# Viictor/vrenderer

Hardware: AMD Instinct MI355X
Metric: shaded Gpixels/s at 8K terrain (higher is better)
Workload: dtype f32

## Files before the change

include/vrterrain.h:

```cpp
#ifndef VRTERRAIN_H
#define VRTERRAIN_H

#include <stddef.h>
#include <stdint.h>

#ifdef __cplusplus
extern "C" {
#endif

#define VR_API __attribute__((visibility("default")))

enum {
    VR_OK = 0,
    VR_ERR_INVALID_ARGUMENT = 1,
    VR_ERR_NO_DEVICE = 2,
    VR_ERR_OUT_OF_MEMORY = 3,
    VR_ERR_TOO_MANY_INSTANCES = 4,
    VR_ERR_OVERFLOW = 5,
    VR_ERR_HIP = 6
};

#define VR_MAX_LODS 12

typedef struct vr_terrain_params {
// ... 236 lines not shown
    const vr_light*         lights;
    int32_t                 num_lights;
    int32_t                 tiled;
    float                   ambient_top[3], ambient_bottom[3];
    const vr_shadow_binding* shadow;
    vr_image*               hdr_out;
    struct vr_tonemap*      tonemap;
    const vr_tonemap_params* tonemap_params;
    float                   frame_time_seconds;
    int32_t                 reserved0;
    void*                   ldr_out;
    size_t                  ldr_capacity;
    void*                   nccl_comm;
    void*                   gathered;
    void*                   ldr_frame;
} vr_frame_desc;
VR_API int vr_frame_submit(vr_terrain* t, vr_gbuffer* gb, const vr_frame_desc* frame);

VR_API int vr_synth_heightmap(vr_context* ctx, int32_t size, uint32_t seed, uint8_t* out_r8);
VR_API int vr_synth_albedo(vr_context* ctx, int32_t size, uint32_t seed,
                           const uint8_t* height_r8, uint8_t* out_srgba8);

VR_API int vr_debug_render_stats(vr_terrain* t, uint32_t out[8]);
VR_API int vr_debug_tile_order(vr_terrain* t, int32_t* out_tiles, uint32_t* out_bin_lengths, int32_t capacity, int32_t* out_count);
VR_API int vr_terrain_memory_bytes(const vr_terrain* t, uint64_t out[4]);
VR_API int vr_debug_download_vertices(vr_terrain* t, uint32_t first, uint32_t count, float* out_xyzw_wxwz);
VR_API int vr_debug_srgb_encode(vr_context* ctx, const float* in, size_t n, uint8_t* out);
VR_API int vr_debug_fastmath_check(vr_context* ctx, unsigned long long out[3]);

#ifdef __cplusplus
}
#endif
#endif
```

vrenderer_amd/capi.py:

```python
import ctypes as C
import os

VR_MAX_LODS = 12
VR_OWNER_TILE = 128

VR_OK = 0
VR_ERR_INVALID_ARGUMENT = 1
VR_ERR_NO_DEVICE = 2
VR_ERR_OUT_OF_MEMORY = 3
VR_ERR_TOO_MANY_INSTANCES = 4
VR_ERR_OVERFLOW = 5
VR_ERR_HIP = 6

VR_LIGHT_DIRECTIONAL = 1
VR_LIGHT_SPOT = 2
VR_LIGHT_POINT = 3
VR_K_COUNT = 19
VR_TONEMAP_BINS = 256
VR_OPT_ASYNC_GEOMETRY = 1
VR_OPT_DISPATCH_EVENTS = 2
VR_OPT_RASTER_TILE = 3
VR_OPT_PLANE_TRACKING = 4
VR_OPT_SCRATCH_WORST_CASE = 5

# ... 101 lines not shown


assert C.sizeof(Instance) == 112
assert C.sizeof(Light) == 64
assert C.sizeof(FrameDesc) == 160

_PKG_DIR = os.path.dirname(os.path.abspath(__file__))
LIB_PATH = os.path.join(_PKG_DIR, "lib", "libvrterrain.so")
if os.environ.get("VRTERRAIN_LIB"):
    LIB_PATH = os.environ["VRTERRAIN_LIB"]

EXPORTS = [
    "vr_context_create", "vr_context_destroy", "vr_context_set_stream", "vr_context_set_option", "vr_context_synchronize",
    "vr_last_error", "vr_version", "vr_build_experiments", "vr_timing_enable", "vr_timing_collect", "vr_timing_kernel_count", "vr_kernel_name", "vr_view_from_camera", "vr_terrain_default_params",
    "vr_render_default_params", "vr_terrain_create", "vr_terrain_destroy", "vr_terrain_num_lods",
    "vr_terrain_lod_ranges", "vr_terrain_download_mip", "vr_terrain_update_heights", "vr_terrain_download_node_heights", "vr_terrain_select", "vr_terrain_render", "vr_terrain_render_lit", "vr_terrain_prepare", "vr_terrain_num_chunks",
    "vr_gbuffer_create", "vr_gbuffer_destroy", "vr_gbuffer_clear", "vr_gbuffer_describe", "vr_gbuffer_plane_known_zero", "vr_gbuffer_region_census",
    "vr_gbuffer_download", "vr_gbuffer_upload", "vr_image_create", "vr_image_destroy",
    "vr_image_device_ptr", "vr_image_download", "vr_image_upload", "vr_ldr_image_create", "vr_ldr_image_destroy", "vr_ldr_image_device_ptr", "vr_ldr_image_capacity", "vr_ldr_image_download", "vr_ldr_image_upload", "vr_deferred_light", "vr_deferred_light_tiled", "vr_deferred_tiled_status", "vr_partition_num_tiles",
    "vr_partition_packed_bytes", "vr_partition_prepare", "vr_frame_detile",
    "vr_shadow_default_params", "vr_shadow_view_setup", "vr_deferred_light_shadowed",
    "vr_tonemap_default_params", "vr_tonemap_create", "vr_tonemap_destroy", "vr_tonemap_reset_exposure", "vr_tonemap_reset_histogram",
    "vr_tonemap_add_frame_to_histogram", "vr_tonemap_histogram_device_ptr", "vr_tonemap_compute_exposure", "vr_tonemap_render",
    "vr_tonemap_simple_render", "vr_tonemap_download", "vr_partition_packed_bytes_ldr", "vr_frame_detile_ldr", "vr_frame_submit", "vr_frame_allgather", "vr_frame_allgather_tiles", "vr_frame_allgather_ldr", "vr_tonemap_allreduce_histogram", "vr_synth_heightmap", "vr_synth_albedo", "vr_debug_srgb_encode", "vr_debug_fastmath_check", "vr_debug_render_stats", "vr_debug_tile_order", "vr_debug_download_vertices", "vr_terrain_memory_bytes",
]

_lib = None


def load_library():
    global _lib
    if _lib is not None:
        return _lib
    if not os.path.exists(LIB_PATH):
        raise RuntimeError(
            f"{LIB_PATH} is missing: the HIP extension has not been built "
            "(run `python -c 'import __graft_entry__ as g; g.build()'`). "
            "vrenderer_amd has no CPU fallback.")
    try:
        import torch
    except Exception:
        pass
    lib = C.CDLL(LIB_PATH, mode=C.RTLD_GLOBAL)
    P = C.POINTER
    vp = C.c_void_p
    sig = {
        "vr_context_create": (C.c_int, [C.c_int, P(vp)]),
# ... 63 lines not shown
        "vr_shadow_default_params": (None, [P(ShadowParams), C.c_float]),
        "vr_shadow_view_setup": (C.c_int, [P(Light), P(View), P(ShadowParams), P(View)]),
        "vr_deferred_light_shadowed": (C.c_int, [vp, P(View), vp, P(Light), C.c_int32, P(C.c_float), P(C.c_float),
                                                 vp, P(Partition), P(ShadowBinding)]),
        "vr_tonemap_default_params": (None, [P(TonemapParams)]),
        "vr_tonemap_create": (C.c_int, [vp, P(vp)]),
        "vr_tonemap_destroy": (None, [vp]),
        "vr_tonemap_reset_exposure": (C.c_int, [vp, C.c_float]),
        "vr_tonemap_reset_histogram": (C.c_int, [vp]),
        "vr_tonemap_add_frame_to_histogram": (C.c_int, [vp, P(TonemapParams), vp, C.c_int32, C.c_int32, P(Partition)]),
        "vr_tonemap_histogram_device_ptr": (vp, [vp]),
        "vr_tonemap_compute_exposure": (C.c_int, [vp, P(TonemapParams), C.c_float]),
        "vr_tonemap_render": (C.c_int, [vp, P(TonemapParams), vp, C.c_int32, C.c_int32, vp, C.c_size_t, P(Partition)]),
        "vr_tonemap_simple_render": (C.c_int, [vp, P(TonemapParams), C.c_float, vp, vp, C.c_size_t]),
        "vr_tonemap_download": (C.c_int, [vp, P(C.c_uint32), P(C.c_float)]),
        "vr_partition_packed_bytes_ldr": (C.c_size_t, [C.c_int32, C.c_int32, C.c_int32]),
        "vr_frame_detile_ldr": (C.c_int, [vp, vp, C.c_int32, C.c_int32, C.c_int32, vp]),
        "vr_synth_heightmap": (C.c_int, [vp, C.c_int32, C.c_uint32, vp]),
        "vr_synth_albedo": (C.c_int, [vp, C.c_int32, C.c_uint32, vp, vp]),
        "vr_debug_srgb_encode": (C.c_int, [vp, vp, C.c_size_t, vp]),
        "vr_debug_fastmath_check": (C.c_int, [vp, vp]),
        "vr_debug_render_stats": (C.c_int, [vp, P(C.c_uint32)]),
        "vr_debug_tile_order": (C.c_int, [vp, vp, vp, C.c_int32, P(C.c_int32)]),
        "vr_debug_download_vertices": (C.c_int, [vp, C.c_uint32, C.c_uint32, vp]),
        "vr_terrain_memory_bytes": (C.c_int, [vp, P(C.c_uint64)]),
    }
    for name in EXPORTS:
        fn = getattr(lib, name)
        fn.restype, fn.argtypes = sig[name]
    _lib = lib
    return lib


class VrError(RuntimeError):
    def __init__(self, code, where):
        msg = ""
        try:
            msg = load_library().vr_last_error().decode()
        except Exception:
            pass
        super().__init__(f"{where} failed with status {code}: {msg}")
        self.code = code


def check(code, where):
    if code != VR_OK:
# ... 2 lines not shown
```

vrenderer_amd/csrc/vr_deferred.hip:

```cpp
#include "vr_internal.h"
#include "vr_tex_dev.h"

#include <math.h>
#include <string.h>

#include "vr_deferred_dev.h"

template <bool PACKED, bool NT = false>
__device__ __forceinline__ void store_quad(uint2* __restrict__ out, size_t out_index, const uint32_t o[8])
{
    if (PACKED) {
        uint2* dst = reinterpret_cast<uint2*>(reinterpret_cast<uint16_t*>(out) + out_index * 3);
        dst[0] = make_uint2(o[0], (o[1] & 0xffffu) | (o[2] << 16));
        dst[1] = make_uint2((o[2] >> 16) | (o[3] << 16), o[4]);
        dst[2] = make_uint2((o[5] & 0xffffu) | (o[6] << 16), (o[6] >> 16) | (o[7] << 16));
    } else {
        uint4* dst = reinterpret_cast<uint4*>(out + out_index);
        if (NT) {
            typedef uint32_t u32x4 __attribute__((ext_vector_type(4)));
            const u32x4 v0 = { o[0], o[1], o[2], o[3] }, v1 = { o[4], o[5], o[6], o[7] };
            __builtin_nontemporal_store(v0, reinterpret_cast<u32x4*>(dst)); __builtin_nontemporal_store(v1, reinterpret_cast<u32x4*>(dst) + 1);
        } else {
            dst[0] = make_uint4(o[0], o[1], o[2], o[3]);
            dst[1] = make_uint4(o[4], o[5], o[6], o[7]);
// ... 41 lines not shown
    const uint4 df = LD16(g_diff + p);
    const uint4 sp = LD16(g_spec + p);
    const uint4 n0 = LD16(g_nrm + p);
    const uint4 n1 = LD16(g_nrm + p + 2);
    const uint4 e0 = LD16(g_emi + p);
    const uint4 e1 = LD16(g_emi + p + 2);
#undef LD16

    const float depth[4] = { dz.x, dz.y, dz.z, dz.w };
    const uint32_t dfa[4] = { df.x, df.y, df.z, df.w }, spa[4] = { sp.x, sp.y, sp.z, sp.w };
    const uint32_t na[8] = { n0.x, n0.y, n0.z, n0.w, n1.x, n1.y, n1.z, n1.w };
    const uint32_t ea[8] = { e0.x, e0.y, e0.z, e0.w, e1.x, e1.y, e1.z, e1.w };
    uint32_t o[8];
#pragma unroll
    for (int k = 0; k < 4; k++) {
        float rgb[3];
        shade_pixel<EXTRA, SHADOW>(a, lut, px0 + k, py, depth[k], dfa[k], spa[k], na[2 * k], na[2 * k + 1], ea[2 * k], ea[2 * k + 1], rgb, &sh);
        o[2 * k] = vr_float_to_half(rgb[0]) | (vr_float_to_half(rgb[1]) << 16);
        o[2 * k + 1] = vr_float_to_half(rgb[2]);
    }
    store_quad<PACKED, NT>(out, out_index, o);
}

template <bool PACKED, bool EXTRA, bool SHADOW = false, bool NT = false>
__global__ __launch_bounds__(256, VR_DEFERRED_WAVES) void k_deferred(DeferredArgs a, const float* __restrict__ g_depth,
                                                   const uint32_t* __restrict__ g_diff, const uint32_t* __restrict__ g_spec,
                                                   const uint2* __restrict__ g_nrm, const uint2* __restrict__ g_emi,
                                                   uint2* __restrict__ out, const float* __restrict__ lut_g,
                                                   const int32_t* __restrict__ owned_tiles, ShadowArgs sh, PlaneHints hints)
{
    __shared__ float lut[256];
    int px0, py;
    size_t out_index;
    bool valid;
    if (PACKED) {
        const int lt = blockIdx.x >> 4, rg = blockIdx.x & 15;
        const int tile = owned_tiles[lt];
        const int ty = tile / a.tiles_x, tx = tile - ty * a.tiles_x;
        const int row = rg * 8 + (threadIdx.x >> 5), col = (threadIdx.x & 31) * 4;
        px0 = tx * VR_OWNER_TILE + col; py = ty * VR_OWNER_TILE + row;
        out_index = ((size_t)lt * VR_OWNER_TILE + row) * VR_OWNER_TILE + col;
        valid = px0 < a.w && py < a.h;
    } else {
        const size_t q = (size_t)blockIdx.x * 256 + threadIdx.x;
        const size_t p = q * 4;
        valid = p < (size_t)a.w * a.h;
        py = (int)(p / (size_t)a.w); px0 = (int)(p - (size_t)py * a.w);
        out_index = p;
    }
    const size_t p = (size_t)py * a.w + px0;
    uint32_t st = 0u;
    if (valid && hints.region != nullptr) st = hints.region[((size_t)(py >> 5) * hints.tiles32_x + (size_t)(px0 >> 5)) * 4 + (size_t)((py & 31) >> 3)];
    const float lut_r = lut_g[threadIdx.x];
    typedef uint32_t u32x4 __attribute__((ext_vector_type(4)));
#define LD16(ptr) ({ u32x4 v_; if (NT) v_ = __builtin_nontemporal_load(reinterpret_cast<const u32x4*>(ptr)); else v_ = *reinterpret_cast<const u32x4*>(ptr); \
                     make_uint4(v_.x, v_.y, v_.z, v_.w); })
    const bool known_clear = st == kRegionClear, known_spec = st == kRegionSpec;
    uint4 dzu = make_uint4(0x3f800000u, 0x3f800000u, 0x3f800000u, 0x3f800000u), df = make_uint4(0u, 0u, 0u, 0u), n0 = df, n1 = df, e0 = df, e1 = df;
    uint4 sp = known_spec ? make_uint4(hints.spec_const, hints.spec_const, hints.spec_const, hints.spec_const) : df;
    if (valid && !known_clear) {
        dzu = LD16(g_depth + p);
        df = LD16(g_diff + p);
        if (!known_spec) sp = LD16(g_spec + p);
        n0 = LD16(g_nrm + p);
        n1 = LD16(g_nrm + p + 2);
        if (!hints.emissive_zero) { e0 = LD16(g_emi + p); e1 = LD16(g_emi + p + 2); }
    }
    lut[threadIdx.x] = lut_r;
    __syncthreads();
    if (!valid) return;
    {
        const uint32_t any = (dzu.x ^ 0x3f800000u) | (dzu.y ^ 0x3f800000u) | (dzu.z ^ 0x3f800000u) | (dzu.w ^ 0x3f800000u)
                           | df.x | df.y | df.z | df.w | sp.x | sp.y | sp.z | sp.w | n0.x | n0.y | n0.z | n0.w | n1.x | n1.y | n1.z | n1.w
                           | e0.x | e0.y | e0.z | e0.w | e1.x | e1.y | e1.z | e1.w;
        if (__all(any == 0u)) {
            const uint32_t z[8] = { 0u, 0u, 0u, 0u, 0u, 0u, 0u, 0u };
            store_quad<PACKED, NT>(out, out_index, z);
            return;
        }
    }
    const float4 dz = make_float4(__uint_as_float(dzu.x), __uint_as_float(dzu.y), __uint_as_float(dzu.z), __uint_as_float(dzu.w));
#undef LD16

    const float depth[4] = { dz.x, dz.y, dz.z, dz.w };
    const uint32_t dfa[4] = { df.x, df.y, df.z, df.w }, spa[4] = { sp.x, sp.y, sp.z, sp.w };
    const uint32_t na[8] = { n0.x, n0.y, n0.z, n0.w, n1.x, n1.y, n1.z, n1.w };
    const uint32_t ea[8] = { e0.x, e0.y, e0.z, e0.w, e1.x, e1.y, e1.z, e1.w };
    uint32_t o[8];
#pragma unroll
    for (int k = 0; k < 4; k++) {
        float rgb[3];
        shade_pixel<EXTRA, SHADOW>(a, lut, px0 + k, py, depth[k], dfa[k], spa[k], na[2 * k], na[2 * k + 1], ea[2 * k], ea[2 * k + 1], rgb, &sh);
        o[2 * k] = vr_float_to_half(rgb[0]) | (vr_float_to_half(rgb[1]) << 16);
        o[2 * k + 1] = vr_float_to_half(rgb[2]);
// ... 66 lines not shown
        VR_REQUIRE(shadow->light_index >= 0 && shadow->light_index < num_lights, "shadow light_index out of range");
        VR_REQUIRE(lights[shadow->light_index].type == VR_LIGHT_DIRECTIONAL, "only a directional light carries the cascaded shadow map");
        VR_REQUIRE(shadow->shadow_map->w == shadow->shadow_map->h && shadow->shadow_map->w == shadow->light_view->viewport_w
                   && shadow->light_view->viewport_h == shadow->light_view->viewport_w, "shadow map must be square and match the light view's viewport");
        VR_REQUIRE(shadow->shadow_map->ctx->device == ctx->device, "shadow map lives on another device");
        for (int i = 0; i < 16; i++) sh.w2c[i] = shadow->light_view->world_to_clip[i];
        { VR_HIP(hipSetDevice(ctx->device)); const int rc = vr_gbuffer_materialise(shadow->shadow_map, ctx->stream); if (rc) return rc; }
        sh.depth = shadow->shadow_map->depth; sh.res = shadow->shadow_map->w; sh.light_index = shadow->light_index;
        sh.bias = shadow->depth_bias; sh.out_of_bounds = lights[shadow->light_index].out_of_bounds_shadow;
    }
    VR_REQUIRE(num_lights >= 0 && num_lights <= kMaxLights, "at most 16 lights (terrain_cb.h:15)");
    VR_REQUIRE(num_lights == 0 || lights, "lights is NULL");
    VR_REQUIRE(view->viewport_w == gb->w && view->viewport_h == gb->h && view->viewport_x == 0 && view->viewport_y == 0,
               "view viewport must cover the G-buffer");
    VR_HIP(hipSetDevice(ctx->device));
    DeferredArgs a;
    bool extra = false;
    { int rc = vr_deferred_make_args(view, gb->w, gb->h, lights, num_lights, amb_top, amb_bottom, &a, &extra); if (rc) return rc; }
    const size_t npx = (size_t)gb->w * gb->h;
    const bool packed = part != nullptr;
    PlaneHints hints;
    { int rc = vr_gbuffer_plane_hints(gb, ctx->stream, &hints); if (rc) return rc; }
    const bool hinted = hints.region != nullptr || hints.emissive_zero != 0;
    VrKernelScope ks(ctx, VR_K_DEFERRED, ctx->stream, true);
    if (packed) {
        const PartTables* pt = nullptr;
        int rc = vr_partition_tables(ctx, gb->w, gb->h, part, &pt);
        if (rc) return rc;
        VR_REQUIRE((size_t)pt->max_owned * VR_OWNER_TILE * VR_OWNER_TILE * 6 <= hdr->capacity_bytes,
                   "hdr_out is smaller than vr_partition_packed_bytes()");
        VR_REQUIRE(gb->w % 4 == 0, "partitioned frames need a width that is a multiple of 4");
        a.tiles_x = (gb->w + VR_OWNER_TILE - 1) / VR_OWNER_TILE;
        if (pt->num_owned > 0) {
            if (!hinted) {
                auto kern = shadow ? k_deferred_stream<true, true, true> : (extra ? k_deferred_stream<true, true> : k_deferred_stream<true, false>);
                VR_LAUNCH_TIMED(ks, kern, dim3((unsigned)pt->num_owned * 16), dim3(256), ctx->stream, a, gb->depth, gb->diffuse,
                                   gb->specular, gb->normals, gb->emissive, (uint2*)hdr->data, ctx->d_srgb_lut, pt->d_owned_tiles, sh);
            } else {
            auto kern = shadow ? k_deferred<true, true, true> : (extra ? k_deferred<true, true> : k_deferred<true, false>);
            VR_LAUNCH_TIMED(ks, kern, dim3((unsigned)pt->num_owned * 16), dim3(256), ctx->stream, a, gb->depth, gb->diffuse,
                               gb->specular, gb->normals, gb->emissive, (uint2*)hdr->data, ctx->d_srgb_lut, pt->d_owned_tiles, sh, hints);
            }
        }
    } else {
        VR_REQUIRE(npx * 8 <= hdr->capacity_bytes, "hdr_out is smaller than the frame");
        if (gb->w % 4 == 0) {
            const size_t quads = npx / 4;
            const bool nt = true;
            if (!hinted) {
                auto kern = shadow ? k_deferred_stream<false, true, true, true> : extra ? k_deferred_stream<false, true, false, true>
                                                                                        : k_deferred_stream<false, false, false, true>;
                VR_LAUNCH_TIMED(ks, kern, dim3((unsigned)((quads + 255) / 256)), dim3(256), ctx->stream, a, gb->depth, gb->diffuse,
                                   gb->specular, gb->normals, gb->emissive, (uint2*)hdr->data, ctx->d_srgb_lut, (const int32_t*)nullptr, sh);
            } else {
            auto kern = shadow ? (nt ? k_deferred<false, true, true, true> : k_deferred<false, true, true, false>)
                               : extra ? (nt ? k_deferred<false, true, false, true> : k_deferred<false, true, false, false>)
                                       : (nt ? k_deferred<false, false, false, true> : k_deferred<false, false, false, false>);
            VR_LAUNCH_TIMED(ks, kern, dim3((unsigned)((quads + 255) / 256)), dim3(256), ctx->stream, a, gb->depth, gb->diffuse,
                               gb->specular, gb->normals, gb->emissive, (uint2*)hdr->data, ctx->d_srgb_lut, (const int32_t*)nullptr, sh, hints);
            }
        } else {
            VR_LAUNCH_TIMED(ks, k_deferred_scalar, dim3((unsigned)((npx + 255) / 256)), dim3(256), ctx->stream, a, gb->depth, gb->diffuse,
                               gb->specular, gb->normals, gb->emissive, (uint2*)hdr->data, ctx->d_srgb_lut, sh, shadow ? 1 : 0);
        }
    }
    VR_HIP(hipGetLastError());
    return VR_OK;
}

extern "C" VR_API int vr_deferred_light(vr_context* ctx, const vr_view* view, vr_gbuffer* gb, const vr_light* lights,
                                         int32_t num_lights, const float amb_top[3], const float amb_bottom[3],
                                         vr_image* hdr, const vr_partition* part)
{
    return deferred_light(ctx, view, gb, lights, num_lights, amb_top, amb_bottom, hdr, part, nullptr);
}

extern "C" VR_API int vr_deferred_light_shadowed(vr_context* ctx, const vr_view* view, vr_gbuffer* gb, const vr_light* lights,
                                                  int32_t num_lights, const float amb_top[3], const float amb_bottom[3],
                                                  vr_image* hdr, const vr_partition* part, const vr_shadow_binding* shadow)
{
    VR_REQUIRE(shadow, "shadow binding is NULL (use vr_deferred_light)");
    return deferred_light(ctx, view, gb, lights, num_lights, amb_top, amb_bottom, hdr, part, shadow);
// ... 339 lines not shown
            o[2 * k + 1] = vr_float_to_half(rgb[2]);
        }
    }
    if (inside) store_quad<PACKED, NT>(out, out_index, o);
}

extern "C" VR_API int vr_deferred_light_tiled(vr_context* ctx, const vr_view* view, vr_gbuffer* gb, const vr_light* lights,
                                               int32_t num_lights, const float amb_top[3], const float amb_bottom[3],
                                               vr_image* hdr, const vr_partition* part)
{
    VR_REQUIRE(ctx && view && gb && hdr && amb_top && amb_bottom, "NULL argument");
    VR_REQUIRE(num_lights >= 0 && num_lights <= 65536 && (num_lights == 0 || lights), "bad light list");
    VR_REQUIRE(view->viewport_w == gb->w && view->viewport_h == gb->h && view->viewport_x == 0 && view->viewport_y == 0,
               "view viewport must cover the G-buffer");
    VR_HIP(hipSetDevice(ctx->device));
    if ((size_t)num_lights > ctx->light_capacity) {
        VR_HIP(hipStreamSynchronize(ctx->stream));
        (void)hipFree(ctx->d_lights); ctx->d_lights = nullptr; ctx->light_capacity = 0; ctx->h_lights_on_device.clear();
        const size_t cap = (size_t)num_lights < 1024 ? 1024 : (size_t)num_lights;
        VR_HIP(hipMalloc(&ctx->d_lights, cap * sizeof(DevLight)));
        ctx->light_capacity = cap;
    }
    if (!ctx->d_flags) { VR_HIP(hipMalloc(&ctx->d_flags, 64)); VR_HIP(hipMemsetAsync(ctx->d_flags, 0, 64, ctx->stream)); }
    PlaneHints hints;
    { const int rc = vr_gbuffer_plane_hints(gb, ctx->stream, &hints); if (rc) return rc; }
    ctx->h_lights.resize((size_t)num_lights);
    for (int i = 0; i < num_lights; i++) { int rc = fill_light(lights[i], ctx->h_lights[i], false); if (rc) return rc; }
    const size_t light_bytes = (size_t)num_lights * sizeof(DevLight);
    if (num_lights && (ctx->h_lights_on_device.size() != (size_t)num_lights
                       || memcmp(ctx->h_lights_on_device.data(), ctx->h_lights.data(), light_bytes) != 0)) {
        ctx->h_lights_on_device.clear();
        VR_HIP(hipMemcpyAsync(ctx->d_lights, ctx->h_lights.data(), light_bytes, hipMemcpyHostToDevice, ctx->stream));
        ctx->h_lights_on_device = ctx->h_lights;
    }
    DeferredArgs a;
    memset(&a, 0, sizeof(a));
    for (int i = 0; i < 16; i++) a.c2w[i] = view->clip_to_world[i];
    for (int i = 0; i < 3; i++) { a.cam[i] = view->camera_pos[i]; a.amb_top[i] = amb_top[i]; a.amb_bot[i] = amb_bottom[i]; }
    a.w = gb->w; a.h = gb->h; a.sx = 2.0f / (float)gb->w; a.sy = -2.0f / (float)gb->h; a.num_lights = 0;
    for (int i = 0; i < num_lights; i++) if (ctx->h_lights[i].type != VR_LIGHT_DIRECTIONAL) a.exact_pos = 1;
    const bool packed = part != nullptr;
    VR_REQUIRE(gb->w % 4 == 0, "the tiled pass needs a frame width that is a multiple of 4");
    const int macro_x = (gb->w + kMacroTile - 1) / kMacroTile, macro_y = (gb->h + kMacroTile - 1) / kMacroTile;
    const int tx = (gb->w + kLightTile - 1) / kLightTile, ty = (gb->h + kLightTile - 1) / kLightTile;
    const int stride = (num_lights < kTileLightCap ? num_lights : kTileLightCap) + 1;
    const size_t words = (size_t)tx * ty * stride;
// ... 63 lines not shown
    }
    return VR_OK;
}

__global__ __launch_bounds__(256) void k_detile(const uint32_t* __restrict__ gathered, uint4* __restrict__ frame, int w, int h,
                                                 int tiles_x, const int32_t* __restrict__ tile_slot)
{
    const size_t i = (size_t)blockIdx.x * 256 + threadIdx.x;
    const size_t p = i * 2;
    if (p >= (size_t)w * h) return;
    const int y = (int)(p / (size_t)w), x = (int)(p - (size_t)y * w);
    const int tx = x / VR_OWNER_TILE, ty = y / VR_OWNER_TILE;
    const int slot = tile_slot[ty * tiles_x + tx];
    const size_t src = ((size_t)slot * VR_OWNER_TILE + (y - ty * VR_OWNER_TILE)) * VR_OWNER_TILE + (x - tx * VR_OWNER_TILE);
    const uint32_t* g = gathered + src * 3 / 2;
    const uint32_t d0 = g[0], d1 = g[1], d2 = g[2];
    frame[i] = make_uint4(d0, d1 & 0xffffu, (d1 >> 16) | (d2 << 16), d2 >> 16);
}

extern "C" VR_API int vr_frame_detile(vr_context* ctx, const void* gathered, int32_t world, vr_image* frame)
{
    VR_REQUIRE(ctx && gathered && frame, "NULL argument");
    VR_REQUIRE(frame->w % 2 == 0 && world >= 1, "frame width must be even");
    VR_HIP(hipSetDevice(ctx->device));
    const PartTables* pt = nullptr;
    { int rc = vr_partition_slot_tables(ctx, frame->w, frame->h, world, &pt); if (rc) return rc; }
    const size_t pairs = (size_t)frame->w * frame->h / 2;
    const int tiles_x = (frame->w + VR_OWNER_TILE - 1) / VR_OWNER_TILE;
    VrKernelScope ks(ctx, VR_K_DETILE);
    hipLaunchKernelGGL(k_detile, dim3((unsigned)((pairs + 255) / 256)), dim3(256), 0, ctx->stream, (const uint32_t*)gathered,
                       (uint4*)frame->data, frame->w, frame->h, tiles_x, pt->d_tile_slot);
    VR_HIP(hipGetLastError());
    return VR_OK;
}
```

vrenderer_amd/csrc/vr_host.hip:

```cpp
#include "vr_internal.h"
#include "vr_experiments.h"

#include <math.h>
#include <stdarg.h>
#include <stdio.h>
#include <string.h>
#include <stdlib.h>

static thread_local char g_last_error[512] = "";
void vr_set_error(const char* fmt, ...)
{
    va_list ap; va_start(ap, fmt);
    vsnprintf(g_last_error, sizeof(g_last_error), fmt, ap);
    va_end(ap);
}
extern "C" VR_API const char* vr_last_error(void) { return g_last_error; }
extern "C" VR_API const char* vr_version(void) { return "vrterrain 0.1 (gfx950)"; }
extern "C" VR_API uint32_t vr_build_experiments(void) { return kExpMask; }

static double srgb_eotf(double c) { return c <= 0.04045 ? c / 12.92 : pow((c + 0.055) / 1.055, 2.4); }

static void timing_reset(vr_context* c);

extern "C" VR_API int vr_context_create(int device, vr_context** out)
// ... 472 lines not shown
    const int rc = vr_gbuffer_region_prepare(g, s, &r);
    if (rc) return rc;
    out->region = r; out->emissive_zero = g->emissive_zero ? 1 : 0;
    return VR_OK;
}

extern "C" VR_API int vr_gbuffer_region_census(vr_gbuffer* g, uint32_t counts[4])
{
    VR_REQUIRE(g && counts, "NULL argument");
    counts[0] = counts[1] = counts[2] = counts[3] = 0;
    const int tiles = ((g->w + 31) / 32) * ((g->h + 31) / 32);
    counts[3] = (uint32_t)tiles * 4u;
    if (!g->ctx->plane_tracking || g->escaped) { counts[0] = counts[3]; return VR_OK; }
    if (g->clear_pending) { counts[2] = counts[3]; return VR_OK; }
    if (!g->d_region || g->region_fill >= 0) { counts[g->region_fill == (int)kRegionClear ? 2 : 0] = counts[3]; return VR_OK; }
    VR_HIP(hipSetDevice(g->ctx->device));
    std::vector<uint8_t> h((size_t)tiles * 4);
    VR_HIP(hipMemcpyAsync(h.data(), g->d_region, h.size(), hipMemcpyDeviceToHost, g->ctx->stream));
    VR_HIP(hipStreamSynchronize(g->ctx->stream));
    for (uint8_t b : h) counts[b <= 2 ? b : 0]++;
    return VR_OK;
}

extern "C" VR_API int vr_gbuffer_plane_known_zero(vr_gbuffer* g, int plane)
{
    if (!g || plane != 4) return 0;
    return (g->ctx->plane_tracking && (g->emissive_zero || g->clear_pending) && !g->escaped) ? 1 : 0;
}

__global__ void k_fill_u32x2(uint2* p, size_t n, uint32_t x, uint32_t y)
{
    for (size_t i = (size_t)blockIdx.x * blockDim.x + threadIdx.x; i < n; i += (size_t)gridDim.x * blockDim.x) p[i] = make_uint2(x, y);
}
int vr_gbuffer_ranges_prepare(vr_gbuffer* g, hipStream_t s)
{
    const int tiles = ((g->w + 31) / 32) * ((g->h + 31) / 32);
    if (!g->d_ranges || g->ranges_tiles != tiles) {
        VR_HIP(hipStreamSynchronize(s));
        (void)hipFree(g->d_ranges); g->d_ranges = nullptr; g->ranges_state = vr_gbuffer::RANGES_NONE;
        VR_HIP(hipMalloc(&g->d_ranges, (size_t)tiles * sizeof(uint2)));
        g->ranges_tiles = tiles;
    }
    if (g->ranges_state != vr_gbuffer::RANGES_CLEAN) {
        hipLaunchKernelGGL(k_fill_u32x2, dim3((unsigned)((tiles + 255) / 256)), dim3(256), 0, s, g->d_ranges, (size_t)tiles, 0x7f800000u, 0u);
        VR_HIP(hipGetLastError());
        g->ranges_state = vr_gbuffer::RANGES_CLEAN;
// ... 57 lines not shown
{
    VR_REQUIRE(ctx && out, "NULL argument");
    VR_REQUIRE(w > 0 && h > 0, "bad image size");
    VR_HIP(hipSetDevice(ctx->device));
    vr_image* im = new vr_image();
    im->ctx = ctx; im->w = w; im->h = h; im->owned = (external == nullptr);
    im->capacity_bytes = (size_t)w * h * 8;
    if (external) im->data = external;
    else {
        hipError_t e = hipMalloc(&im->data, im->capacity_bytes);
        if (e != hipSuccess) { delete im; vr_set_error("hipMalloc(%zu) failed", (size_t)w * h * 8); return VR_ERR_OUT_OF_MEMORY; }
    }
    *out = im;
    return VR_OK;
}
extern "C" VR_API void vr_image_destroy(vr_image* im)
{
    if (!im) return;
    (void)hipSetDevice(im->ctx->device);
    if (im->read_pending) (void)hipEventSynchronize(im->ev_read_done);
    if (im->ev_written) (void)hipEventDestroy(im->ev_written);
    if (im->ev_read_done) (void)hipEventDestroy(im->ev_read_done);
    if (im->owned) (void)hipFree(im->data);
    delete im;
}
extern "C" VR_API void* vr_image_device_ptr(vr_image* im) { return im ? im->data : nullptr; }
extern "C" VR_API int vr_image_download(vr_image* im, void* host, size_t bytes)
{
    VR_REQUIRE(im && host, "NULL argument");
    VR_REQUIRE(bytes <= im->capacity_bytes, "byte count exceeds the image");
    VR_HIP(hipSetDevice(im->ctx->device));
    VR_HIP(hipMemcpyAsync(host, im->data, bytes, hipMemcpyDeviceToHost, im->ctx->stream));
    VR_HIP(hipStreamSynchronize(im->ctx->stream));
    return VR_OK;
}

extern "C" VR_API int vr_image_upload(vr_image* im, const void* host, size_t bytes)
{
    VR_REQUIRE(im && host, "NULL argument");
    VR_REQUIRE(bytes <= im->capacity_bytes, "byte count exceeds the image");
    VR_HIP(hipSetDevice(im->ctx->device));
    VR_HIP(hipMemcpyAsync(im->data, host, bytes, hipMemcpyHostToDevice, im->ctx->stream));
    VR_HIP(hipStreamSynchronize(im->ctx->stream));
    return VR_OK;
}

extern "C" VR_API int vr_ldr_image_create(vr_context* ctx, int32_t w, int32_t h, size_t capacity_bytes, void* external, vr_ldr_image** out)
{
    VR_REQUIRE(ctx && out, "NULL argument");
    VR_REQUIRE(w > 0 && h > 0, "bad image size");
    VR_HIP(hipSetDevice(ctx->device));
    const size_t cap = capacity_bytes ? capacity_bytes : (size_t)w * h * 4;
    void* data = external;
    if (!external) {
        hipError_t e = hipMalloc(&data, cap);
        if (e != hipSuccess) { vr_set_error("hipMalloc(%zu) failed: %s", cap, hipGetErrorString(e)); return VR_ERR_OUT_OF_MEMORY; }
    }
    vr_ldr_image* im = new vr_ldr_image();
    im->ctx = ctx; im->w = w; im->h = h; im->data = data; im->owned = external == nullptr; im->capacity_bytes = cap;
    *out = im;
    return VR_OK;
}
extern "C" VR_API void vr_ldr_image_destroy(vr_ldr_image* im)
{
// ... 145 lines not shown
```

vrenderer_amd/csrc/vr_internal.h:

```cpp
#pragma once

#include <hip/hip_runtime.h>
#include <hip/hip_ext.h>
#include <stdint.h>
#include <stdlib.h>
#include <string>
#include <vector>

#include "../../include/vrterrain.h"

void vr_set_error(const char* fmt, ...);
#define VR_HIP(expr)                                                                  \
    do {                                                                              \
        hipError_t e__ = (expr);                                                      \
        if (e__ != hipSuccess) {                                                      \
            vr_set_error("%s:%d: %s -> %s", __FILE__, __LINE__, #expr, hipGetErrorString(e__)); \
            return e__ == hipErrorOutOfMemory ? VR_ERR_OUT_OF_MEMORY : VR_ERR_HIP;    \
        }                                                                             \
    } while (0)
#define VR_REQUIRE(cond, msg)                                                         \
    do { if (!(cond)) { vr_set_error("%s:%d: %s", __FILE__, __LINE__, msg); return VR_ERR_INVALID_ARGUMENT; } } while (0)

constexpr int kGrid = 32;
constexpr int kSide = kGrid + 1;
// ... 122 lines not shown
    uint2* d_ranges = nullptr;
    int ranges_tiles = 0;
    enum { RANGES_NONE = 0, RANGES_CLEAN, RANGES_VALID, RANGES_DIRTY };
    int ranges_state = RANGES_NONE;
    int ranges_rank = 0, ranges_world = 1;
    bool emissive_zero = false;
    bool escaped = false;
    uint8_t* d_region = nullptr;
    int region_tiles = 0;
    int region_fill = 0;
    bool clear_pending = false;
    bool cleared_once = false;
};
int vr_gbuffer_materialise(vr_gbuffer* g, hipStream_t s);
constexpr uint32_t kRegionSpec = 1u, kRegionClear = 2u;
int vr_gbuffer_region_prepare(vr_gbuffer* g, hipStream_t s, uint8_t** out);
struct PlaneHints {
    const uint8_t* region;
    uint32_t spec_const;
    int emissive_zero;
    int tiles32_x;
};
int vr_gbuffer_plane_hints(vr_gbuffer* g, hipStream_t s, PlaneHints* out);
uint32_t vr_specular_constant(const vr_context* c);
inline void vr_gbuffer_touch(vr_gbuffer* g) { if (g->ranges_state == vr_gbuffer::RANGES_VALID) g->ranges_state = vr_gbuffer::RANGES_DIRTY; }
int vr_gbuffer_ranges_prepare(vr_gbuffer* g, hipStream_t s);

struct vr_image {
    vr_context* ctx;
    int w, h;
    void* data;
    bool owned;
    size_t capacity_bytes;
    hipEvent_t ev_written = nullptr, ev_read_done = nullptr;
    bool read_pending = false;
};

struct vr_ldr_image {
    vr_context* ctx;
    int w, h;
    void* data;
    bool owned;
    size_t capacity_bytes;
};

constexpr int kGeoSets = 3;
struct GeoSet {
    uint32_t* d_node_ids = nullptr;
    vr_instance* d_instances = nullptr;
    uint32_t* d_counters = nullptr;
    uint32_t* d_sel_scratch = nullptr;
    DevVert* d_verts = nullptr;
    uint64_t* d_rect = nullptr;
    uint4* d_recs = nullptr;
    uint32_t* d_hard_list = nullptr;
    HardTriRec* d_hard_tris = nullptr;
    uint32_t* d_hard_first = nullptr;
    uint32_t* d_tile_count = nullptr;
    uint32_t* d_tile_offset = nullptr;
// ... 97 lines not shown
```

vrenderer_amd/csrc/vr_raster.hip:

```cpp
#include "vr_internal.h"
#include "vr_tex_dev.h"
#include "vr_deferred_dev.h"
#include "vr_experiments.h"
#include <type_traits>

#include <stdlib.h>
#include <string.h>

struct VertexArgs {
    float w2v[16], v2c[16];
    float cam_x, cam_z;
    float lod_ranges[VR_MAX_LODS];
    float morph_start, world_size, max_height;
    float vp_x, vp_y, vp_w, vp_h;
};

struct RasterArgs {
    int w, h;
    int vx0, vy0, vx1, vy1;
    int rtx, rty;
    int tile_shift;
    int mirrored;
    int world, rank;
    uint32_t world_magic;
// ... 1641 lines not shown
        const uint64_t span = (uint64_t)((const char*)(gb->emissive + (size_t)gb->w * gb->h) - (const char*)gb->depth);
        const bool one_rsrc = (const char*)gb->depth < (const char*)gb->diffuse && (const char*)gb->depth < (const char*)gb->specular
                           && (const char*)gb->depth < (const char*)gb->normals && (const char*)gb->depth < (const char*)gb->emissive && span < (1ull << 32);
        const bool fast = same && a.ws_pow2 && one_rsrc && !a.wireframe && !a.depth_only;
        const bool depth = a.depth_only && !a.wireframe;
        const bool ranges = rp->depth_ranges && fast && a.assume_cleared && !gb->escaped;
        if (ranges) {
            if ((rc = vr_gbuffer_ranges_prepare(gb, s))) return rc;
            gb->ranges_state = vr_gbuffer::RANGES_VALID; gb->ranges_rank = a.rank; gb->ranges_world = a.world;
        } else vr_gbuffer_touch(gb);
        const bool noemi = fast && ctx->plane_tracking && gb->emissive_zero && !gb->escaped;
        auto kern = a.tile_shift == 5 ? pick_raster<32>(a.wireframe != 0, fast, depth, ranges, noemi) : pick_raster<64>(a.wireframe != 0, fast, depth, ranges, noemi);
        LitArgs la;
        bool fuse = false;
        if (lit_req && fast && !ranges) {
            bool extra = false;
            memset(&la, 0, sizeof(la));
            if ((rc = vr_deferred_make_args(view, gb->w, gb->h, lit_req->lights, lit_req->num_lights, lit_req->amb_top, lit_req->amb_bottom, &la.da, &extra))) return rc;
            VR_REQUIRE(view->viewport_w == gb->w && view->viewport_h == gb->h && view->viewport_x == 0 && view->viewport_y == 0,
                       "view viewport must cover the G-buffer");
            fuse = !extra && gb->w % 4 == 0;
            if (fuse) {
                la.lut_g = ctx->d_srgb_lut; la.hdr = (uint2*)lit_req->hdr->data;
                if (pt) {
                    VR_REQUIRE((size_t)pt->max_owned * VR_OWNER_TILE * VR_OWNER_TILE * 6 <= lit_req->hdr->capacity_bytes, "hdr_out is smaller than vr_partition_packed_bytes()");
                    la.tile_slot = pt->d_tile_slot; la.slot_base = pt->rank * pt->max_owned; la.owner_tiles_x = (gb->w + VR_OWNER_TILE - 1) / VR_OWNER_TILE;
                    la.da.tiles_x = la.owner_tiles_x;
                } else VR_REQUIRE((size_t)gb->w * gb->h * 8 <= lit_req->hdr->capacity_bytes, "hdr_out is smaller than the frame");
            }
        }
        if (lit_done) *lit_done = fuse;
        uint8_t* region = nullptr;
        if (fast && !fuse && a.tile_shift == 5 && ctx->plane_tracking && !gb->escaped) { if ((rc = vr_gbuffer_region_prepare(gb, s, &region))) return rc; }
        else gb->region_fill = 0;
#define VR_RASTER_ARGS a, t->height, t->albedo, g.d_verts, g.d_hard_tris, g.d_hard_first, \
                           (const uint4*)g.d_recs, (uint32_t)t->cap_instances * (uint32_t)kTrisPerInst, g.d_tile_cursor, g.d_tile_offset, g.d_bin_entries, tiles, g.d_counters + C_CLASS0, \
                           gb->depth, gb->diffuse, gb->specular, gb->normals, gb->emissive, ctx->d_srgb_thr, ctx->d_enc_tab, spec_const, ranges ? gb->d_ranges : (uint2*)nullptr, region
        if (fuse) {
            ks.id = VR_K_RASTER_LIT;
            if (a.tile_shift == 5) VR_LAUNCH_TIMED(ks, (k_raster<false, 32, RM_FAST, false, true, true>), dim3(grid), dim3(kRT), s, VR_RASTER_ARGS, la);
            else VR_LAUNCH_TIMED(ks, (k_raster<false, 64, RM_FAST, false, true, true>), dim3(grid), dim3(kRT), s, VR_RASTER_ARGS, la);
        } else
        VR_LAUNCH_TIMED(ks, kern, dim3(grid), dim3(kRT), s, VR_RASTER_ARGS, LitNone());
#undef VR_RASTER_ARGS
        if (ctx->dispatch_events && ks.e0 && ks.e1) pass_stop = ks.e1;
        if (!fuse && !noemi && !a.depth_only && a.assume_cleared && a.world <= 1) gb->emissive_zero = true;
// ... 42 lines not shown
```

vrenderer_amd/passes.py:

```python
import ctypes as C

import numpy as np

from . import capi
from .capi import (GBufferDesc, Instance, Light, Partition, RenderParams, TerrainParams, View, check)


def _vp(a):
    return a.ctypes.data_as(C.c_void_p)


def _f3(v):
    return (C.c_float * 3)(*[float(x) for x in v])


class Context:

    def __init__(self, device=0):
        self.lib = capi.load_library()
        h = C.c_void_p()
        check(self.lib.vr_context_create(device, C.byref(h)), "vr_context_create")
        self.handle = h
        self.device = device

# ... 105 lines not shown

    def __init__(self, ctx):
        self.ctx = ctx
        self.handle = None
        self.width = self.height = 0

    def Init(self, width, height):
        self.close()
        h = C.c_void_p()
        check(self.ctx.lib.vr_gbuffer_create(self.ctx.handle, width, height, C.byref(h)), "vr_gbuffer_create")
        self.handle, self.width, self.height = h, width, height
        return self

    def Clear(self):
        check(self.ctx.lib.vr_gbuffer_clear(self.handle), "vr_gbuffer_clear")

    def plane_known_zero(self, plane="emissive"):
        return bool(self.ctx.lib.vr_gbuffer_plane_known_zero(self.handle, self.PLANES[plane][0]))

    def region_census(self):
        c = (C.c_uint32 * 4)()
        check(self.ctx.lib.vr_gbuffer_region_census(self.handle, c), "vr_gbuffer_region_census")
        return dict(unknown=c[0], specular_constant=c[1], clear=c[2], total=c[3])

    def describe(self):
        d = GBufferDesc()
        check(self.ctx.lib.vr_gbuffer_describe(self.handle, C.byref(d)), "vr_gbuffer_describe")
        return d

    def download(self, plane):
        idx, dt, tail = self.PLANES[plane]
        out = np.empty((self.height, self.width) + tail, dt)
        check(self.ctx.lib.vr_gbuffer_download(self.handle, idx, _vp(out), out.nbytes), "vr_gbuffer_download")
        return out

    def upload(self, plane, arr):
        idx, dt, tail = self.PLANES[plane]
        a = np.ascontiguousarray(arr, dt)
        assert a.shape == (self.height, self.width) + tail
        check(self.ctx.lib.vr_gbuffer_upload(self.handle, idx, _vp(a), a.nbytes), "vr_gbuffer_upload")

    def close(self):
        if self.handle:
            self.ctx.lib.vr_gbuffer_destroy(self.handle)
            self.handle = None

# ... 422 lines not shown
```

Measured before the change: 78.71.

## Classify deferred-shading waves by region state and skip redundant clear-pixel stores

After: 75.74. 0.962x the previous value.

```diff
diff --git a/include/vrterrain.h b/include/vrterrain.h
--- a/include/vrterrain.h
+++ b/include/vrterrain.h
@@ -282,6 +282,7 @@
                            const uint8_t* height_r8, uint8_t* out_srgba8);
 
 VR_API int vr_debug_render_stats(vr_terrain* t, uint32_t out[8]);
+VR_API int vr_debug_region_states(vr_gbuffer* gb, uint8_t* out, size_t capacity);
 VR_API int vr_debug_tile_order(vr_terrain* t, int32_t* out_tiles, uint32_t* out_bin_lengths, int32_t capacity, int32_t* out_count);
 VR_API int vr_terrain_memory_bytes(const vr_terrain* t, uint64_t out[4]);
 VR_API int vr_debug_download_vertices(vr_terrain* t, uint32_t first, uint32_t count, float* out_xyzw_wxwz);
diff --git a/vrenderer_amd/capi.py b/vrenderer_amd/capi.py
--- a/vrenderer_amd/capi.py
+++ b/vrenderer_amd/capi.py
@@ -147,7 +147,7 @@
     "vr_shadow_default_params", "vr_shadow_view_setup", "vr_deferred_light_shadowed",
     "vr_tonemap_default_params", "vr_tonemap_create", "vr_tonemap_destroy", "vr_tonemap_reset_exposure", "vr_tonemap_reset_histogram",
     "vr_tonemap_add_frame_to_histogram", "vr_tonemap_histogram_device_ptr", "vr_tonemap_compute_exposure", "vr_tonemap_render",
-    "vr_tonemap_simple_render", "vr_tonemap_download", "vr_partition_packed_bytes_ldr", "vr_frame_detile_ldr", "vr_frame_submit", "vr_frame_allgather", "vr_frame_allgather_tiles", "vr_frame_allgather_ldr", "vr_tonemap_allreduce_histogram", "vr_synth_heightmap", "vr_synth_albedo", "vr_debug_srgb_encode", "vr_debug_fastmath_check", "vr_debug_render_stats", "vr_debug_tile_order", "vr_debug_download_vertices", "vr_terrain_memory_bytes",
+    "vr_tonemap_simple_render", "vr_tonemap_download", "vr_partition_packed_bytes_ldr", "vr_frame_detile_ldr", "vr_frame_submit", "vr_frame_allgather", "vr_frame_allgather_tiles", "vr_frame_allgather_ldr", "vr_tonemap_allreduce_histogram", "vr_synth_heightmap", "vr_synth_albedo", "vr_debug_srgb_encode", "vr_debug_fastmath_check", "vr_debug_render_stats", "vr_debug_tile_order", "vr_debug_region_states", "vr_debug_download_vertices", "vr_terrain_memory_bytes",
 ]
 
 _lib = None
@@ -257,6 +257,7 @@
         "vr_debug_fastmath_check": (C.c_int, [vp, vp]),
         "vr_debug_render_stats": (C.c_int, [vp, P(C.c_uint32)]),
         "vr_debug_tile_order": (C.c_int, [vp, vp, vp, C.c_int32, P(C.c_int32)]),
+        "vr_debug_region_states": (C.c_int, [vp, vp, C.c_size_t]),
         "vr_debug_download_vertices": (C.c_int, [vp, C.c_uint32, C.c_uint32, vp]),
         "vr_terrain_memory_bytes": (C.c_int, [vp, P(C.c_uint64)]),
     }
diff --git a/vrenderer_amd/csrc/vr_deferred.hip b/vrenderer_amd/csrc/vr_deferred.hip
--- a/vrenderer_amd/csrc/vr_deferred.hip
+++ b/vrenderer_amd/csrc/vr_deferred.hip
@@ -87,17 +87,36 @@
     store_quad<PACKED, NT>(out, out_index, o);
 }
 
+constexpr uint32_t kWaveMixed = 0u;
+constexpr uint32_t kWaveClear = 1u;
+constexpr uint32_t kWaveTerrain = 2u;
+constexpr uint32_t kWaveNone = 3u;
+__device__ __forceinline__ uint32_t wave_class(const PlaneHints& hints, uint32_t row, uint32_t segx)
+{
+    const uint32_t* __restrict__ w = reinterpret_cast<const uint32_t*>(hints.region) + ((size_t)(row >> 5) * (uint32_t)hints.tiles32_x + (size_t)segx * 8u);
+    const uint32_t shift = ((row & 31u) >> 3) * 8u;
+    uint32_t not_clear = 0u, not_spec = 0u;
+#pragma unroll
+    for (int j = 0; j < 8; j++) { const uint32_t b = (w[j] >> shift) & 255u; not_clear |= b ^ kRegionClear; not_spec |= b ^ kRegionSpec; }
+    return not_clear == 0u ? kWaveClear : (not_spec == 0u && hints.emissive_zero != 0) ? kWaveTerrain : kWaveMixed;
+}
+
 template <bool PACKED, bool EXTRA, bool SHADOW = false, bool NT = false>
 __global__ __launch_bounds__(256, VR_DEFERRED_WAVES) void k_deferred(DeferredArgs a, const float* __restrict__ g_depth,
                                                    const uint32_t* __restrict__ g_diff, const uint32_t* __restrict__ g_spec,
                                                    const uint2* __restrict__ g_nrm, const uint2* __restrict__ g_emi,
                                                    uint2* __restrict__ out, const float* __restrict__ lut_g,
-                                                   const int32_t* __restrict__ owned_tiles, ShadowArgs sh, PlaneHints hints)
+                                                   const int32_t* __restrict__ owned_tiles, ShadowArgs sh, PlaneHints hints, WaveStates ws)
 {
     __shared__ float lut[256];
+    constexpr bool WAVE = !PACKED && !EXTRA && !SHADOW;
     int px0, py;
     size_t out_index;
     bool valid;
+    uint32_t cls = kWaveMixed;
+    uint32_t zbyte = 0u;
+    uint32_t seg = 0u;
+    const bool waves = WAVE && ws.enabled != 0;
     if (PACKED) {
         const int lt = blockIdx.x >> 4, rg = blockIdx.x & 15;
         const int tile = owned_tiles[lt];
@@ -106,6 +125,33 @@
         px0 = tx * VR_OWNER_TILE + col; py = ty * VR_OWNER_TILE + row;
         out_index = ((size_t)lt * VR_OWNER_TILE + row) * VR_OWNER_TILE + col;
         valid = px0 < a.w && py < a.h;
+    } else if (waves) {
+        const uint32_t wv = __builtin_amdgcn_readfirstlane(threadIdx.x >> 6);
+        const uint32_t segs_x = (uint32_t)a.w >> 8, nseg = segs_x * (uint32_t)a.h;
+        const uint32_t seg0 = blockIdx.x * 4u;
+        const uint32_t zr = ws.zero_rows != nullptr ? reinterpret_cast<const uint32_t*>(ws.zero_rows)[blockIdx.x] : 0u;
+        uint32_t row = seg0 / segs_x, segx = seg0 - row * segs_x, my_row = 0u, my_segx = 0u;
+        bool nothing_to_shade = true;
+#pragma unroll
+        for (uint32_t j = 0; j < 4u; j++) {
+            const uint32_t c = seg0 + j < nseg ? wave_class(hints, row, segx) : kWaveNone;
+            nothing_to_shade = nothing_to_shade && (c == kWaveClear || c == kWaveNone);
+            if (j == wv) { cls = c; my_row = row; my_segx = segx; }
+            if (++segx == segs_x) { segx = 0u; row++; }
+        }
+        seg = seg0 + wv;
+        zbyte = (zr >> (8u * wv)) & 255u;
+        py = (int)my_row; px0 = (int)(my_segx * 256u + (threadIdx.x & 63u) * 4u);
+        out_index = (size_t)seg * 256u + (threadIdx.x & 63u) * 4u;
+        valid = cls != kWaveNone;
+        if (nothing_to_shade) {
+            if (cls == kWaveClear && zbyte != 1u) {
+                const uint32_t z[8] = { 0u, 0u, 0u, 0u, 0u, 0u, 0u, 0u };
+                store_quad<PACKED, NT>(out, out_index, z);
+                if (ws.zero_rows != nullptr && (threadIdx.x & 63u) == 0u) ws.zero_rows[seg] = 1;
+            }
+            return;
+        }
     } else {
         const size_t q = (size_t)blockIdx.x * 256 + threadIdx.x;
         const size_t p = q * 4;
@@ -115,7 +161,7 @@
     }
     const size_t p = (size_t)py * a.w + px0;
     uint32_t st = 0u;
-    if (valid && hints.region != nullptr) st = hints.region[((size_t)(py >> 5) * hints.tiles32_x + (size_t)(px0 >> 5)) * 4 + (size_t)((py & 31) >> 3)];
+    if (cls == kWaveMixed && valid && hints.region != nullptr) st = hints.region[((size_t)(py >> 5) * hints.tiles32_x + (size_t)(px0 >> 5)) * 4 + (size_t)((py & 31) >> 3)];
     const float lut_r = lut_g[threadIdx.x];
     typedef uint32_t u32x4 __attribute__((ext_vector_type(4)));
 #define LD16(ptr) ({ u32x4 v_; if (NT) v_ = __builtin_nontemporal_load(reinterpret_cast<const u32x4*>(ptr)); else v_ = *reinterpret_cast<const u32x4*>(ptr); \
@@ -123,7 +169,13 @@
     const bool known_clear = st == kRegionClear, known_spec = st == kRegionSpec;
     uint4 dzu = make_uint4(0x3f800000u, 0x3f800000u, 0x3f800000u, 0x3f800000u), df = make_uint4(0u, 0u, 0u, 0u), n0 = df, n1 = df, e0 = df, e1 = df;
     uint4 sp = known_spec ? make_uint4(hints.spec_const, hints.spec_const, hints.spec_const, hints.spec_const) : df;
-    if (valid && !known_clear) {
+    if (waves && cls == kWaveTerrain) {
+        sp = make_uint4(hints.spec_const, hints.spec_const, hints.spec_const, hints.spec_const);
+        dzu = LD16(g_depth + p);
+        df = LD16(g_diff + p);
+        n0 = LD16(g_nrm + p);
+        n1 = LD16(g_nrm + p + 2);
+    } else if (cls == kWaveMixed && valid && !known_clear) {
         dzu = LD16(g_depth + p);
         df = LD16(g_diff + p);
         if (!known_spec) sp = LD16(g_spec + p);
@@ -134,7 +186,16 @@
     lut[threadIdx.x] = lut_r;
     __syncthreads();
     if (!valid) return;
-    {
+    if (waves && cls == kWaveClear) {
+        if (zbyte != 1u) {
+            const uint32_t z[8] = { 0u, 0u, 0u, 0u, 0u, 0u, 0u, 0u };
+            store_quad<PACKED, NT>(out, out_index, z);
+            if (ws.zero_rows != nullptr && (threadIdx.x & 63u) == 0u) ws.zero_rows[seg] = 1;
+        }
+        return;
+    }
+    if (waves && ws.zero_rows != nullptr && zbyte != 0u && (threadIdx.x & 63u) == 0u) ws.zero_rows[seg] = 0;
+    if (!(waves && cls == kWaveTerrain)) {
         const uint32_t any = (dzu.x ^ 0x3f800000u) | (dzu.y ^ 0x3f800000u) | (dzu.z ^ 0x3f800000u) | (dzu.w ^ 0x3f800000u)
                            | df.x | df.y | df.z | df.w | sp.x | sp.y | sp.z | sp.w | n0.x | n0.y | n0.z | n0.w | n1.x | n1.y | n1.z | n1.w
                            | e0.x | e0.y | e0.z | e0.w | e1.x | e1.y | e1.z | e1.w;
@@ -247,6 +308,11 @@
     PlaneHints hints;
     { int rc = vr_gbuffer_plane_hints(gb, ctx->stream, &hints); if (rc) return rc; }
     const bool hinted = hints.region != nullptr || hints.emissive_zero != 0;
+    WaveStates ws = { nullptr, 0 };
+    if (!packed && !shadow && !extra && gb->w % 256 == 0 && hints.region != nullptr) {
+        ws.enabled = 1;
+        const int rc = vr_image_zero_rows(hdr, gb->w, gb->h, ctx->stream, &ws.zero_rows); if (rc) return rc;
+    } else vr_image_written(hdr);
     VrKernelScope ks(ctx, VR_K_DEFERRED, ctx->stream, true);
     if (packed) {
         const PartTables* pt = nullptr;
@@ -264,7 +330,7 @@
             } else {
             auto kern = shadow ? k_deferred<true, true, true> : (extra ? k_deferred<true, true> : k_deferred<true, false>);
             VR_LAUNCH_TIMED(ks, kern, dim3((unsigned)pt->num_owned * 16), dim3(256), ctx->stream, a, gb->depth, gb->diffuse,
-                               gb->specular, gb->normals, gb->emissive, (uint2*)hdr->data, ctx->d_srgb_lut, pt->d_owned_tiles, sh, hints);
+                               gb->specular, gb->normals, gb->emissive, (uint2*)hdr->data, ctx->d_srgb_lut, pt->d_owned_tiles, sh, hints, ws);
             }
         }
     } else {
@@ -282,7 +348,7 @@
                                : extra ? (nt ? k_deferred<false, true, false, true> : k_deferred<false, true, false, false>)
                                        : (nt ? k_deferred<false, false, false, true> : k_deferred<false, false, false, false>);
             VR_LAUNCH_TIMED(ks, kern, dim3((unsigned)((quads + 255) / 256)), dim3(256), ctx->stream, a, gb->depth, gb->diffuse,
-                               gb->specular, gb->normals, gb->emissive, (uint2*)hdr->data, ctx->d_srgb_lut, (const int32_t*)nullptr, sh, hints);
+                               gb->specular, gb->normals, gb->emissive, (uint2*)hdr->data, ctx->d_srgb_lut, (const int32_t*)nullptr, sh, hints, ws);
             }
         } else {
             VR_LAUNCH_TIMED(ks, k_deferred_scalar, dim3((unsigned)((npx + 255) / 256)), dim3(256), ctx->stream, a, gb->depth, gb->diffuse,
@@ -668,6 +734,7 @@
         ctx->light_capacity = cap;
     }
     if (!ctx->d_flags) { VR_HIP(hipMalloc(&ctx->d_flags, 64)); VR_HIP(hipMemsetAsync(ctx->d_flags, 0, 64, ctx->stream)); }
+    vr_image_written(hdr);
     PlaneHints hints;
     { const int rc = vr_gbuffer_plane_hints(gb, ctx->stream, &hints); if (rc) return rc; }
     ctx->h_lights.resize((size_t)num_lights);
@@ -777,6 +844,7 @@
 {
     VR_REQUIRE(ctx && gathered && frame, "NULL argument");
     VR_REQUIRE(frame->w % 2 == 0 && world >= 1, "frame width must be even");
+    vr_image_written(frame);
     VR_HIP(hipSetDevice(ctx->device));
     const PartTables* pt = nullptr;
     { int rc = vr_partition_slot_tables(ctx, frame->w, frame->h, world, &pt); if (rc) return rc; }
diff --git a/vrenderer_amd/csrc/vr_host.hip b/vrenderer_amd/csrc/vr_host.hip
--- a/vrenderer_amd/csrc/vr_host.hip
+++ b/vrenderer_amd/csrc/vr_host.hip
@@ -518,6 +518,20 @@
     return VR_OK;
 }
 
+extern "C" VR_API int vr_debug_region_states(vr_gbuffer* g, uint8_t* out, size_t capacity)
+{
+    VR_REQUIRE(g && out, "NULL argument");
+    const size_t n = (size_t)((g->w + 31) / 32) * ((g->h + 31) / 32) * 4;
+    VR_REQUIRE(capacity >= n, "capacity is smaller than the region array");
+    if (!g->ctx->plane_tracking || g->escaped) { memset(out, 0, n); return VR_OK; }
+    if (g->clear_pending) { memset(out, (int)kRegionClear, n); return VR_OK; }
+    if (!g->d_region || g->region_fill >= 0) { memset(out, g->region_fill > 0 ? g->region_fill : 0, n); return VR_OK; }
+    VR_HIP(hipSetDevice(g->ctx->device));
+    VR_HIP(hipMemcpyAsync(out, g->d_region, n, hipMemcpyDeviceToHost, g->ctx->stream));
+    VR_HIP(hipStreamSynchronize(g->ctx->stream));
+    return VR_OK;
+}
+
 extern "C" VR_API int vr_gbuffer_plane_known_zero(vr_gbuffer* g, int plane)
 {
     if (!g || plane != 4) return 0;
@@ -621,9 +635,34 @@
     if (im->ev_written) (void)hipEventDestroy(im->ev_written);
     if (im->ev_read_done) (void)hipEventDestroy(im->ev_read_done);
     if (im->owned) (void)hipFree(im->data);
+    if (im->d_zero_rows) (void)hipFree(im->d_zero_rows);
     delete im;
 }
-extern "C" VR_API void* vr_image_device_ptr(vr_image* im) { return im ? im->data : nullptr; }
+extern "C" VR_API void* vr_image_device_ptr(vr_image* im)
+{
+    if (!im) return nullptr;
+    im->escaped = true; im->zero_rows_valid = false;
+    return im->data;
+}
+
+int vr_image_zero_rows(vr_image* im, int w, int h, hipStream_t s, uint8_t** out)
+{
+    *out = nullptr;
+    if (!im->owned || im->escaped) { im->zero_rows_valid = false; return VR_OK; }
+    if (!im->d_zero_rows) {
+        const size_t bytes = ((im->capacity_bytes / (8 * 256) + 3) & ~(size_t)3) + 4;
+        VR_HIP(hipMalloc(&im->d_zero_rows, bytes));
+        im->zero_rows_bytes = bytes; im->zero_rows_valid = false;
+    }
+    const size_t need = ((((size_t)w >> 8) * (size_t)h + 3) & ~(size_t)3);
+    VR_REQUIRE(need <= im->zero_rows_bytes, "image is smaller than the frame");
+    if (!im->zero_rows_valid || im->zero_w != w || im->zero_h != h || im->zero_stream != s) {
+        VR_HIP(hipMemsetAsync(im->d_zero_rows, 0, need, s));
+        im->zero_rows_valid = true; im->zero_w = w; im->zero_h = h; im->zero_stream = s;
+    }
+    *out = im->d_zero_rows;
+    return VR_OK;
+}
 extern "C" VR_API int vr_image_download(vr_image* im, void* host, size_t bytes)
 {
     VR_REQUIRE(im && host, "NULL argument");
@@ -639,6 +678,7 @@
     VR_REQUIRE(im && host, "NULL argument");
     VR_REQUIRE(bytes <= im->capacity_bytes, "byte count exceeds the image");
     VR_HIP(hipSetDevice(im->ctx->device));
+    vr_image_written(im);
     VR_HIP(hipMemcpyAsync(im->data, host, bytes, hipMemcpyHostToDevice, im->ctx->stream));
     VR_HIP(hipStreamSynchronize(im->ctx->stream));
     return VR_OK;
diff --git a/vrenderer_amd/csrc/vr_internal.h b/vrenderer_amd/csrc/vr_internal.h
--- a/vrenderer_amd/csrc/vr_internal.h
+++ b/vrenderer_amd/csrc/vr_internal.h
@@ -168,6 +168,10 @@
     int tiles32_x;
 };
 int vr_gbuffer_plane_hints(vr_gbuffer* g, hipStream_t s, PlaneHints* out);
+struct WaveStates {
+    uint8_t* zero_rows;
+    int enabled;
+};
 uint32_t vr_specular_constant(const vr_context* c);
 inline void vr_gbuffer_touch(vr_gbuffer* g) { if (g->ranges_state == vr_gbuffer::RANGES_VALID) g->ranges_state = vr_gbuffer::RANGES_DIRTY; }
 int vr_gbuffer_ranges_prepare(vr_gbuffer* g, hipStream_t s);
@@ -180,7 +184,14 @@
     size_t capacity_bytes;
     hipEvent_t ev_written = nullptr, ev_read_done = nullptr;
     bool read_pending = false;
-};
+    uint8_t* d_zero_rows = nullptr;
+    size_t zero_rows_bytes = 0;
+    bool zero_rows_valid = false, escaped = false;
+    int zero_w = 0, zero_h = 0;
+    hipStream_t zero_stream = nullptr;
+};
+inline void vr_image_written(vr_image* im) { im->zero_rows_valid = false; }
+int vr_image_zero_rows(vr_image* im, int w, int h, hipStream_t s, uint8_t** out);
 
 struct vr_ldr_image {
     vr_context* ctx;
diff --git a/vrenderer_amd/csrc/vr_raster.hip b/vrenderer_amd/csrc/vr_raster.hip
--- a/vrenderer_amd/csrc/vr_raster.hip
+++ b/vrenderer_amd/csrc/vr_raster.hip
@@ -1687,6 +1687,7 @@
             fuse = !extra && gb->w % 4 == 0;
             if (fuse) {
                 la.lut_g = ctx->d_srgb_lut; la.hdr = (uint2*)lit_req->hdr->data;
+                vr_image_written(lit_req->hdr);
                 if (pt) {
                     VR_REQUIRE((size_t)pt->max_owned * VR_OWNER_TILE * VR_OWNER_TILE * 6 <= lit_req->hdr->capacity_bytes, "hdr_out is smaller than vr_partition_packed_bytes()");
                     la.tile_slot = pt->d_tile_slot; la.slot_base = pt->rank * pt->max_owned; la.owner_tiles_x = (gb->w + VR_OWNER_TILE - 1) / VR_OWNER_TILE;
diff --git a/vrenderer_amd/passes.py b/vrenderer_amd/passes.py
--- a/vrenderer_amd/passes.py
+++ b/vrenderer_amd/passes.py
@@ -151,6 +151,12 @@
         c = (C.c_uint32 * 4)()
         check(self.ctx.lib.vr_gbuffer_region_census(self.handle, c), "vr_gbuffer_region_census")
         return dict(unknown=c[0], specular_constant=c[1], clear=c[2], total=c[3])
+
+    def region_states(self):
+        ty, tx = (self.height + 31) // 32, (self.width + 31) // 32
+        out = np.zeros((ty, tx, 4), np.uint8)
+        check(self.ctx.lib.vr_debug_region_states(self.handle, _vp(out), out.nbytes), "vr_debug_region_states")
+        return out
 
     def describe(self):
         d = GBufferDesc()
```
